# cure-lab/PnPInversion

Measured on AMD Instinct MI355X. Metric: edited images/sec @ 512x512, 50 DDIM-inv + 50 denoise steps, higher is better.
Workload: dtype f16 (fp32 accumulate; latents / scheduler math fp32); 1 GPU; single 512x512 image per rank, SD-1.x (seeded synthetic weights), directinversion+p2p, faithful schedule: 650 UNet sample-forwards + 1 VAE encode + 5 VAE decodes per image, Refine+Reweight+LocalBlend controller; text K/V projected once per loop (not per forward); ddim_steps=50, schedule=lockstep

## Files before the change

pnpinversion_amd/csrc/api.hip:

```cpp
#include <math.h>
#include <stdio.h>
#include <stdlib.h>
#include <string.h>

#include <algorithm>
#include <functional>
#include <memory>
#include <string>

#include "model.h"

static int g_text_kv = 1;
static int g_temb_cache = 1;

static int fail(pnpi_ctx* c, int status, const char* what) {
  c->err = what;
  return status;
}
static int fail_launch(pnpi_ctx* c, int code, const char* what) {
  char buf[640];
  if (code > 0) {
    snprintf(buf, sizeof(buf), "HIP error %d (%s) in %s", code, hipGetErrorString((hipError_t)code), what);
    c->err = buf;
    return PNPI_EHIP;
// ... 587 lines not shown
    half_t* f = talloc(c, (size_t)M * t.I);
    CK(op_gemm(c, h2, H, M, H, L.fc1.w, H, t.I, L.fc1.b, nullptr, 0, f, t.I));
    if (!c->dry) CK(launch_quick_gelu(f, (size_t)M * t.I, c->st));
    CK(op_gemm(c, f, t.I, M, t.I, L.fc2.w, t.I, H, L.fc2.b, x1, H, x, H));
    c->temp.release(mk);
  }
  half_t* y = palloc(c, (size_t)M * H);
  if (!c->dry) {
    PROF(PNPI_KC_LAYERNORM, 0.0, 2.0 * M * (double)H * 2.0, launch_layernorm(x, M, H, 1e-5f, t.final_ln.g, t.final_ln.b, y, c->st));
    CK(launch_f16_to_f32(y, (size_t)M * H, out, c->st));
  }
  return 0;
}

int pnpi_text_encode(pnpi_ctx* c, const int32_t* input_ids, int n, float* hidden_out) {
  if (!c || !input_ids || !hidden_out || n <= 0) return PNPI_EINVAL;
  CKP(check_clip_ready(c));
  if (n > c->rows_ident_n) return fail(c, PNPI_EINVAL, "more prompts than max(max_unet_rows, 8)");
  return clip_fwd(c, (const int*)input_ids, n, hidden_out);
}

static int conv_hook(pnpi_ctx* c, const void* x1, const void* x2, int C1, int C2, int B, int H, int W, int ksize, int stride, int pad, int ups,
                     int Ho, int Wo, const void* w, const float* bias, const void* res, int N, void* out, int force_cfg, int force_split,
                     float* stats_out, int* tile_rows_out) {
  GemmP p; gemm_defaults(p);
  p.x1 = (const half_t*)x1; p.x2 = (const half_t*)x2; p.C1 = C1; p.C2 = C2; p.ldx1 = C1; p.ldx2 = C2;
  p.B = B; p.H = H; p.W = W; p.Ho = Ho; p.Wo = Wo; p.ksize = ksize; p.stride = stride; p.pad = pad; p.ups = ups;
  p.K = ksize * ksize * (C1 + C2); p.w = (const half_t*)w; p.ldw = p.K; p.M = B * Ho * Wo; p.N = N;
  p.bias = bias; p.res = (const half_t*)res; p.ldres = N; p.out = (half_t*)out; p.ldo = N; p.stats = stats_out;
  CK(launch_igemm(p, c->splitk_ws, c->splitk_bytes, c->st, force_cfg, force_split, nullptr, tile_rows_out));
  return 0;
}
int pnpi_op_conv(pnpi_ctx* c, const void* x1, const void* x2, int C1, int C2, int B, int H, int W, int ksize, int stride, int pad,
                 int ups, int Ho, int Wo, const void* w, const float* bias, const void* res, int N, void* out, int force_cfg,
                 int force_split) {
  return conv_hook(c, x1, x2, C1, C2, B, H, W, ksize, stride, pad, ups, Ho, Wo, w, bias, res, N, out, force_cfg, force_split, nullptr, nullptr);
}
int pnpi_op_conv_stats(pnpi_ctx* c, const void* x1, const void* x2, int C1, int C2, int B, int H, int W, int ksize, int stride, int pad,
                       int ups, int Ho, int Wo, const void* w, const float* bias, const void* res, int N, void* out, int force_cfg,
                       int force_split, float* stats_out, int* tile_rows_out) {
  if (!c || !stats_out || !tile_rows_out) return PNPI_EINVAL;
  return conv_hook(c, x1, x2, C1, C2, B, H, W, ksize, stride, pad, ups, Ho, Wo, w, bias, res, N, out, force_cfg, force_split, stats_out, tile_rows_out);
}
int pnpi_tile_table_lookup(int M, int N, int K, int ksize, int* cfg, int* split, int* entry_m) {
  return igemm_table_lookup(M, N, K, ksize, cfg, split, entry_m);
}
int pnpi_set_tuning(const char* key, int value) {
  if (!key) return PNPI_EINVAL;
  if (!strcmp(key, "text_kv")) { g_text_kv = value; return 0; }
  if (!strcmp(key, "temb_cache")) { g_temb_cache = value; return 0; }
  if (!strcmp(key, "gn_inline_rows")) { norm_set_tuning_gn_inline_rows(value); return 0; }
  if (!strcmp(key, "attn_vt_perm")) { g_vt_perm = value; return 0; }
  if (!strcmp(key, "attn_aug")) { g_attn_aug = value; return 0; }
  if (!strcmp(key, "attn_pipe")) return attn_set_tuning_pipe(value) == 0 ? 0 : PNPI_EINVAL;
  if (!strcmp(key, "gn_slab")) { g_gn_slab = value; return 0; }
  if (!strcmp(key, "op_attention_aug")) { g_op_attention_aug = value; return 0; }
  if (!strcmp(key, "op_attention_vt_perm")) { g_op_attention_vt_perm = value; return 0; }
  if (!strcmp(key, "attn_bwd_flash")) { g_attn_bwd_flash = value; return 0; }
  return igemm_set_tuning(key, value) == 0 ? 0 : PNPI_EINVAL;
}
int pnpi_op_gemm(pnpi_ctx* c, const void* a, int lda, const void* w, int ldw, int M, int N, int K, float alpha, const float* bias,
                 const void* res, void* out, int ldo, int vt_col0, void* outT, int vt_ld, int vt_f32, int rpb, int force_cfg,
                 int force_split) {
  GemmP p; gemm_defaults(p);
  p.x1 = (const half_t*)a; p.C1 = K; p.ldx1 = lda; p.B = 1; p.H = 1; p.W = M; p.Ho = 1; p.Wo = M; p.ksize = 1;
  p.w = (const half_t*)w; p.ldw = ldw; p.M = M; p.N = N; p.K = K; p.alpha = alpha; p.bias = bias; p.res = (const half_t*)res;
  p.ldres = N; p.out = (half_t*)out; p.ldo = ldo;
  if (outT) { p.outT = outT; p.vt_col0 = vt_col0; p.vt_ld = vt_ld; p.vt_f32 = vt_f32; p.rows_per_batch = rpb; }
  CK(launch_igemm(p, c->splitk_ws, c->splitk_bytes, c->st, force_cfg, force_split));
  return 0;
}
int pnpi_op_gemm_geglu(pnpi_ctx* c, const void* a, int lda, const void* w, int ldw, int M, int N, int K, const float* bias, void* out,
                       int ldo) {
  GemmP p; gemm_defaults(p);
  p.x1 = (const half_t*)a; p.C1 = K; p.ldx1 = lda; p.B = 1; p.H = 1; p.W = M; p.Ho = 1; p.Wo = M; p.ksize = 1;
  p.w = (const half_t*)w; p.ldw = ldw; p.M = M; p.N = N; p.K = K; p.bias = bias; p.out = (half_t*)out; p.ldo = ldo; p.geglu = 1;
  CK(launch_igemm(p, c->splitk_ws, c->splitk_bytes, c->st));
  return 0;
}
int pnpi_op_groupnorm(pnpi_ctx* c, const void* x1, const void* x2, int C1, int C2, int B, int HW, int G, float eps, const float* gamma,
                      const float* beta, int silu, void* out) {
  CK(launch_groupnorm((const half_t*)x1, (const half_t*)x2, C1, C2, B, HW, G, eps, gamma, beta, silu, (half_t*)out, c->gn_partial, c->st));
  return 0;
}
int pnpi_op_layernorm(pnpi_ctx* c, const void* x, int M, int C, float eps, const float* gamma, const float* beta, void* out) {
  CK(launch_layernorm((const half_t*)x, M, C, eps, gamma, beta, (half_t*)out, c->st));
  return 0;
}
int pnpi_op_geglu(pnpi_ctx* c, const void* x, int M, int inner, void* out) {
  CK(launch_geglu((const half_t*)x, M, inner, (half_t*)out, c->st));
  return 0;
}
int pnpi_op_softmax_rows(pnpi_ctx* c, void* x, int M, int N, int ld) {
  CK(launch_softmax_rows((half_t*)x, M, N, ld, c->st));
  return 0;
}
int pnpi_op_attention_bwd(pnpi_ctx* c, const void* q, int ldq, int q_off, const void* k, int ldk, int k_off, const void* v, int ldv, int v_off,
                          const void* d_o, int ldo, int heads, int Nq, int Nk, int Dp, int dh, float scale, int B, void* dq, void* dk, void* dv,
                          void* scratch, size_t scratch_bytes) {
  if (!c || !q || !k || !v || !d_o || !dq || !dk || !dv) return PNPI_EINVAL;
  CKP(attn_bwd(c, (const half_t*)q, ldq, q_off, (const half_t*)k, ldk, k_off, (const half_t*)v, ldv, v_off, (const half_t*)d_o, ldo,
               heads, Nq, Nk, Dp, dh, scale, B, (half_t*)dq, (half_t*)dk, (half_t*)dv, scratch, scratch_bytes));
  return 0;
}
size_t pnpi_op_attention_bwd_scratch_bytes(int Nq, int Nk, int dh) { return attn_bwd_scratch_bytes(Nq, Nk, dh); }
int pnpi_op_layernorm_bwd(pnpi_ctx* c, const void* x, const void* dy, int M, int C, float eps, const float* gamma, void* dx) {
// ... 1 lines not shown
  return 0;
}
int pnpi_op_groupnorm_bwd(pnpi_ctx* c, const void* x1, const void* x2, int C1, int C2, int B, int HW, int G, float eps, const float* gamma,
                          const float* beta, int silu, const void* dy, void* dx) {
  const int C = C1 + C2;
  if (!(C & 7) && !(C1 & 7) && G <= 64) {
    float* ws = nullptr;
    CKP(gn_bwd_workspace(c, B, HW, G, &ws));
    CK(launch_groupnorm_bwd2((const half_t*)x1, (const half_t*)x2, C1, C2, B, HW, G, eps, gamma, beta, silu, (const half_t*)dy,
                             GnbOut{(half_t*)dx, C, 0}, GnbOut{(half_t*)dx + C1, C, 0}, ws, c->st));
    return 0;
  }
  CK(launch_groupnorm_bwd((const half_t*)x1, (const half_t*)x2, C1, C2, B, HW, G, eps, gamma, beta, silu, (const half_t*)dy, (half_t*)dx, c->st));
  return 0;
}
int pnpi_op_geglu_bwd(pnpi_ctx* c, const void* h, const void* dy, int M, int inner, void* dh) {
  CK(launch_geglu_bwd((const half_t*)h, (const half_t*)dy, M, inner, (half_t*)dh, c->st));
  return 0;
}
int pnpi_op_softmax_bwd_rows(pnpi_ctx* c, const float* P, const float* dP, int R, int N, int ld, float scale, void* dS) {
  CK(launch_softmax_bwd_rows(P, dP, (size_t)R, N, ld, scale, (half_t*)dS, c->st));
  return 0;
}
int pnpi_op_accumulate(pnpi_ctx* c, void* dst, const void* src, size_t n) {
  CK(launch_accumulate_f16((half_t*)dst, (const half_t*)src, n, c->st));
  return 0;
}
int pnpi_op_sumpool2x2(pnpi_ctx* c, const void* dup, int B, int H, int W, int C, void* dx) {
  CK(launch_sumpool2x2((const half_t*)dup, B, H, W, C, (half_t*)dx, c->st));
  return 0;
}
int pnpi_op_zero_stuff2(pnpi_ctx* c, const void* dy, int B, int Ho, int Wo, int C, void* out) {
  CK(launch_zero_stuff2((const half_t*)dy, B, Ho, Wo, C, (half_t*)out, c->st));
  return 0;
}
int pnpi_op_repack_dgrad(pnpi_ctx* c, const void* w, int N, int taps, int Cin, void* wd) {
  CK(launch_repack_dgrad((const half_t*)w, N, N, taps, Cin, (half_t*)wd, c->st));
  return 0;
}
int pnpi_op_null_text_loss(pnpi_ctx* c, const float* eps_u, const float* eps_c, const float* x, const float* target, int n, float w, float c_x,
                           float c_e, float grad_scale, void* d_eps_u, float* loss) {
  CK(launch_null_text_loss(eps_u, eps_c, x, target, n, w, c_x, c_e, grad_scale, (float*)d_eps_u, loss, c->st));
  return 0;
}
int pnpi_op_adam_step(pnpi_ctx* c, float* p, float* m, float* v, const float* g, int n, int k, float lr, float inv_scale) {
  CK(launch_adam_step(p, m, v, g, n, k, lr, inv_scale, c->st));
  return 0;
}
int pnpi_op_attention(pnpi_ctx* c, const void* q, int ldq, int q_off, const void* k, int ldk, int k_off, const void* vt, int ldv,
                      void* o, int ldo, int heads, int Nq, int Nk, int Dp, int dh, float scale, const int* rows_dev, int nrows) {
  AttnP a; a.q = (const half_t*)q; a.ldq = ldq; a.q_off = q_off; a.k = (const half_t*)k; a.ldk = ldk; a.k_off = k_off;
  a.vt = (const half_t*)vt; a.ldv = ldv; a.o = (half_t*)o; a.ldo = ldo; a.heads = heads; a.Nq = Nq; a.Nk = Nk; a.Dp = Dp; a.dh = dh;
  a.scale = scale; a.rows = rows_dev; a.nrows = nrows;
  a.vt_perm = (g_op_attention_vt_perm && attn_flash_uses_dma64(Dp, Nk, 0)) ? 1 : 0;
  a.aug = g_op_attention_aug;
  CK(launch_attn_flash(a, c->st));
  return 0;
}
int pnpi_op_cross_edit(pnpi_ctx* c, const void* q, int ldq, int q_off, const void* k, int ldk, int k_off, const void* vt, int ldv,
                       void* o, int ldo, int heads, int Nq, int Nk, int Dp, int dh, float scale, const int* pairs_dev, int npairs,
                       const void* mmatT, const float* c1, const float* c2, const float* lb_alpha, float* lb_acc, int lb_slot0,
                       int lb_nslots) {
  CrossEditP e; e.q = (const half_t*)q; e.ldq = ldq; e.q_off = q_off; e.k = (const half_t*)k; e.ldk = ldk; e.k_off = k_off;
  e.vt = (const half_t*)vt; e.ldv = ldv; e.o = (half_t*)o; e.ldo = ldo; e.heads = heads; e.Nq = Nq; e.Nk = Nk; e.Dp = Dp; e.dh = dh;
  e.scale = scale; e.pairs = pairs_dev; e.npairs = npairs; e.mmatT = (const half_t*)mmatT; e.c1 = c1; e.c2 = c2;
  e.lb_alpha = lb_alpha; e.lb_acc = lb_acc; e.lb_slot0 = lb_slot0; e.lb_nslots = lb_nslots; e.write_src = 1;
  CK(launch_attn_cross_edit(e, c->st));
  return 0;
}
int pnpi_op_local_blend(pnpi_ctx* c, const float* lb_acc, int nslots, int map_hw, int lat_hw, int C, float th, float* latents, int nimg) {
  CK(launch_local_blend(lb_acc, nslots, map_hw, lat_hw, C, th, latents, nimg, c->st));
  return 0;
}
int pnpi_op_local_blend_sub(pnpi_ctx* c, const float* lb_acc, int nslots, int map_hw, int lat_hw, int C, float th, float th_sub,
                            float* latents, int nimg) {
  CK(launch_local_blend(lb_acc, nslots, map_hw, lat_hw, C, th, latents, nimg, c->st, 4, th_sub));
  return 0;
}

#include "api_loops.inc"

}
```

pnpinversion_amd/csrc/api_graph.inc:

```
static void prof_open(pnpi_ctx* c, ProfRec& r) {
  (void)hipEventCreate(&r.a); (void)hipEventCreate(&r.b);
  (void)hipEventRecord(r.a, c->st);
}
static void prof_close(pnpi_ctx* c, ProfRec& r, int cls, double flops, double bytes, int M = 0, int N = 0, int K = 0, int ks = 0) {
  (void)hipEventRecord(r.b, c->st);
  r.cls = cls; r.flops = flops; r.bytes = bytes; r.M = M; r.N = N; r.K = K; r.ksize = ks;
  c->prof.push_back(r);
}
static int g_gn_slab = 0;
static int flush_pending(pnpi_ctx* c) {
  if (!c->pend_on) return 0;
  c->pend_on = false;
  return launch_splitk_reduce(c->pend, c->st);
}
#define PROF(cls, flops, bytes, expr) PROFD(cls, flops, bytes, 0, 0, 0, expr)
#define PROFD(cls, flops, bytes, d0, d1, d2, expr)            \
  do {                                                        \
    if (c->pend_on) { int _f = flush_pending(c); if (_f) return fail_launch(c, _f, "deferred split-K combine"); } \
    if (c->prof_on && !c->dry) {                              \
      ProfRec _pr; prof_open(c, _pr);                         \
      int _r = (expr);                                        \
      prof_close(c, _pr, (cls), (flops), (bytes), (d0), (d1), (d2)); \
      if (_r) return fail_launch(c, _r, #expr);               \
    } else {                                                  \
// ... 173 lines not shown
  if (!keep_acts(c)) c->temp.release(mk);
  return 0;
}

static int attn_materialized(pnpi_ctx* c, const half_t* q, int ldq, int q_off, const half_t* k, int ldk, int k_off, const half_t* vt, int ldv,
                             half_t* o, int ldo, int heads, int Nq, int Nk, int Dp, int dh, float scale, int B, int is_cross, int place,
                             int layer) {
  const int ldp = round_up_i(Nk, 8);
  const size_t need = align_up((size_t)B * heads * Nq * Nk * sizeof(float), 256);
  if (!c->attn_buf || need + (size_t)Nq * ldp * sizeof(half_t) > c->attn_buf_bytes)
    return fail(c, PNPI_ENOMEM, "attention callback buffer too small for this site (rows*heads*Nq*Nk floats + Nq*Nk halfs)");
  half_t* p16 = reinterpret_cast<half_t*>(reinterpret_cast<char*>(c->attn_buf) + need);
  for (int b = 0; b < B; ++b)
    for (int h = 0; h < heads; ++h) {
      float* S = c->attn_buf + ((size_t)b * heads + h) * Nq * Nk;
      VtOut v; v.outT = S; v.col0 = 0; v.ld = Nk; v.f32 = 1; v.rpb = Nk;
      CK(op_gemm(c, k + (size_t)b * Nk * ldk + k_off + h * Dp, ldk, Nk, Dp, q + (size_t)b * Nq * ldq + q_off + h * Dp, ldq, Nq, nullptr,
                 nullptr, 0, nullptr, Nq, scale, &v));
    }
  CK(launch_softmax_rows_f32(c->attn_buf, (size_t)B * heads * Nq, Nk, c->st));
  CKH(hipStreamSynchronize(c->st));
  if (c->attn_cb(c->attn_cb_user, c->attn_buf, B, heads, Nq, Nk, is_cross, place, layer)) return fail(c, PNPI_ESTATE, "attention callback failed");
  for (int b = 0; b < B; ++b)
    for (int h = 0; h < heads; ++h) {
      const float* S = c->attn_buf + ((size_t)b * heads + h) * Nq * Nk;
      CK(launch_f32_rows_to_f16_padded(S, Nq, Nk, ldp, p16, c->st));
      CK(op_gemm(c, p16, ldp, Nq, ldp, vt + ((size_t)b * heads + h) * Dp * (size_t)ldv, ldv, dh, nullptr, nullptr, 0,
                 o + (size_t)b * Nq * ldo + h * dh, ldo));
    }
  return 0;
}

static int transformer_fwd(pnpi_ctx* c, const TransformerW& t, const half_t* x, int B, int H, int W, const half_t* ctx16,
                           bool use_ctrl, int cur_step, half_t* out, Stats sx = Stats(), Stats* so = nullptr) {
  const pnpi_model_config& g = c->cfg;
  const size_t mk = c->temp.mark();
  const int block_index = c->tf_index++;
  const int C = t.C, N = H * W, M = B * N, hd = t.heads * t.Dp, X = g.cross_dim, T = g.ctx_len;
  const float scale = 1.0f / sqrtf((float)t.dh);
  CtrlDev& cd = c->cd;
  const bool edit = use_ctrl && cd.any_edit;

  half_t* g0 = talloc(c, (size_t)M * C);
  CK(op_gn(c, x, nullptr, C, 0, B, N, t.gn, g.norm_groups, 1e-6f, 0, g0, sx));
  half_t* hs = talloc(c, (size_t)M * C);
  CK(op_conv(c, g0, C, nullptr, 0, B, H, W, t.proj_in, 1, 0, 0, t.proj_in.b, nullptr, hs, H, W));

  half_t* n1 = talloc(c, (size_t)M * C);
  if (!c->dry) PROF(PNPI_KC_LAYERNORM, 0.0, 2.0 * M * (double)C * 2.0, launch_layernorm(hs, M, C, 1e-5f, t.ln1.g, t.ln1.b, n1, c->st));
  half_t* qk = talloc(c, (size_t)M * 2 * hd);
  const int ldv = round_up_i(N, 8);
  half_t* vt = talloc(c, (size_t)B * hd * ldv);
  if (c->attn_cb && !c->dry && ldv != N) CKH(hipMemsetAsync(vt, 0, (size_t)B * hd * ldv * sizeof(half_t), c->st));
  const int vperm = (g_vt_perm && !c->attn_cb && N % 16 == 0 && attn_flash_uses_dma64(t.Dp, N, 0)) ? 1 : 0;
  {
    VtOut v; v.outT = vt; v.col0 = 2 * hd; v.ld = ldv; v.f32 = 0; v.rpb = N; v.perm16 = vperm;
    CK(op_gemm(c, n1, C, M, C, t.w_qkv, C, 3 * hd, t.b_qkv_aug, nullptr, 0, qk, 2 * hd, 1.f, &v, 2.0 * M * 3.0 * C * C));
  }
  half_t* ao = talloc(c, (size_t)M * C);
  {
    AttnP a; a.q = qk; a.ldq = 2 * hd; a.q_off = 0; a.k = qk; a.ldk = 2 * hd; a.k_off = hd; a.vt = vt; a.ldv = ldv; a.vt_perm = vperm;
    a.aug = (t.b_qkv_aug && g_attn_aug) ? 1 : 0;
    a.o = ao; a.ldo = C; a.heads = t.heads; a.Nq = N; a.Nk = N; a.Dp = t.Dp; a.dh = t.dh; a.scale = scale;
    const bool rep = edit && cur_step >= cd.self_lo && cur_step < cd.self_hi && N <= cd.self_max_tokens;
    const bool masa_step = cd.masa_step_list ? (cur_step >= 0 && cur_step < (int)cd.masa_step_on.size() && cd.masa_step_on[cur_step]) : cur_step >= cd.masa_start_step;
    const bool masa_layer = cd.masa_layer_mask ? ((cd.masa_layer_mask >> block_index) & 1u) != 0 && block_index < 31 : block_index >= cd.masa_start_layer;
    const bool masa = use_ctrl && cd.masa_any && masa_step && masa_layer;
    a.rows = rep ? cd.rows_rep : (masa ? cd.rows_masa : cd.rows_id); a.nrows = B;
    c->ctr.executed_attn_flops += 4.0 * B * t.heads * (double)N * N * t.Dp;
    if (c->attn_cb && !c->dry) {
      CKP(attn_materialized(c, qk, 2 * hd, 0, qk, 2 * hd, hd, vt, ldv, ao, C, t.heads, N, N, t.Dp, t.dh, scale, B, 0, t.place, 2 * block_index));
    } else if (!c->dry) PROFD(PNPI_KC_ATTN_FLASH, 4.0 * B * t.heads * (double)N * N * t.dh, 0.0, N, N, t.Dp, launch_attn_flash(a, c->st));
  }
  half_t* hs1 = talloc(c, (size_t)M * C);
  CK(op_gemm(c, ao, C, M, C, t.o1.w, C, C, t.o1.b, hs, C, hs1, C));

  half_t* n2 = talloc(c, (size_t)M * C);
  if (!c->dry) PROF(PNPI_KC_LAYERNORM, 0.0, 2.0 * M * (double)C * 2.0, launch_layernorm(hs1, M, C, 1e-5f, t.ln2.g, t.ln2.b, n2, c->st));
  half_t* q2 = talloc(c, (size_t)M * hd);
  CK(op_gemm(c, n2, C, M, C, t.w_q2, C, hd, nullptr, nullptr, 0, q2, hd, 1.f, nullptr, 2.0 * M * (double)C * C));
  const int ldv2 = round_up_i(T, 8);
  half_t *k2, *vt2;
  if (c->tkv.use) {
    k2 = c->tkv.k[block_index]; vt2 = c->tkv.vt[block_index];
  } else {
    k2 = talloc(c, (size_t)B * T * hd);
    vt2 = talloc(c, (size_t)B * hd * ldv2);
    if (c->attn_cb && !c->dry && ldv2 != T) CKH(hipMemsetAsync(vt2, 0, (size_t)B * hd * ldv2 * sizeof(half_t), c->st));
    VtOut v; v.outT = vt2; v.col0 = hd; v.ld = ldv2; v.f32 = 0; v.rpb = T;
    CK(op_gemm(c, ctx16, X, B * T, X, t.w_kv2, X, 2 * hd, nullptr, nullptr, 0, k2, hd, 1.f, &v, 2.0 * B * T * 2.0 * C * X));
  }
  half_t* ao2 = talloc(c, (size_t)M * C);
  {
    AttnP a; a.q = q2; a.ldq = hd; a.q_off = 0; a.k = k2; a.ldk = hd; a.k_off = 0; a.vt = vt2; a.ldv = ldv2;
    a.o = ao2; a.ldo = C; a.heads = t.heads; a.Nq = N; a.Nk = T; a.Dp = t.Dp; a.dh = t.dh; a.scale = scale;
    a.rows = edit ? cd.rows_plain : cd.rows_id; a.nrows = edit ? cd.n_plain : B;
    c->ctr.executed_attn_flops += 4.0 * B * t.heads * (double)N * 96 * t.Dp;
    if (c->attn_cb && !c->dry) {
      CKP(attn_materialized(c, q2, hd, 0, k2, hd, 0, vt2, ldv2, ao2, C, t.heads, N, T, t.Dp, t.dh, scale, B, 1, t.place, 2 * block_index + 1));
    } else if (!c->dry) PROFD(PNPI_KC_ATTN_FLASH, 4.0 * a.nrows * t.heads * (double)N * T * t.dh, 0.0, N, T, t.Dp, launch_attn_flash(a, c->st));
    if (edit && !c->dry && !c->attn_cb) {
      CrossEditP e; e.q = q2; e.ldq = hd; e.q_off = 0; e.k = k2; e.ldk = hd; e.k_off = 0; e.vt = vt2; e.ldv = ldv2;
      e.o = ao2; e.ldo = C; e.heads = t.heads; e.Nq = N; e.Nk = T; e.Dp = t.Dp; e.dh = t.dh; e.scale = scale;
      e.pairs = cd.pairs; e.npairs = cd.npairs; e.mmatT = cd.mmatT;
      int srow = cur_step < cd.n_alpha_rows ? cur_step : cd.n_alpha_rows - 1;
      e.c1 = cd.coef + ((size_t)srow * 2 + 0) * cd.npairs * 96;
      e.c2 = cd.coef + ((size_t)srow * 2 + 1) * cd.npairs * 96;
// ... 379 lines not shown
```

pnpinversion_amd/csrc/attn.hip:

```cpp
#include <stdlib.h>

#include "ops.h"

static constexpr int KV_TILE = 64;
static constexpr int SV_LD = KV_TILE + 4;

template <int DP, bool PF>
__global__ void __launch_bounds__(256) attn_flash_kernel(AttnP p) {
  constexpr int KS = DP / 16;
  constexpr int OT = DP / 32;
  constexpr int SK_LD = DP + 8;
  __shared__ __attribute__((aligned(16))) half_t sK[KV_TILE * SK_LD];
  __shared__ __attribute__((aligned(16))) half_t sV[DP * SV_LD];

  const int tid = threadIdx.x, lane = tid & 63, wave = tid >> 6;
  const int h = lane >> 5, ql = lane & 31;
  const int nqt = (p.Nq + 127) >> 7, T = nqt * p.heads * p.nrows, per = (T + 7) >> 3;
  const int tix = (int)(blockIdx.x & 7) * per + (int)(blockIdx.x >> 3);
  if (tix >= T) return;
  const int qt = tix % nqt, head = (tix / nqt) % p.heads;
  const int* rw = p.rows + (tix / (nqt * p.heads)) * 4;
  const int orow = rw[0], qrow = rw[1], krow = rw[2], vrow = rw[3];
  const int qtok = qt * 128 + wave * 32 + ql;
  const bool qok = qtok < p.Nq;
// ... 104 lines not shown
    }
    const float mc = mrun * c;
    float psum = 0.f;
    half8 pf[2][2];
#pragma unroll
    for (int st = 0; st < 2; ++st)
#pragma unroll
      for (int r = 0; r < 16; ++r) {
        float pv = __builtin_amdgcn_exp2f(__builtin_fmaf(s[st][r], c, -mc));
        psum += pv;
        pf[st][r >> 3][r & 7] = (half_t)pv;
      }
    lrun += psum;
#pragma unroll
    for (int ot = 0; ot < OT; ++ot) {
#pragma unroll
      for (int st = 0; st < 2; ++st)
#pragma unroll
        for (int t = 0; t < 2; ++t) {
          const half_t* vb = sV + (ot * 32 + ql) * SV_LD + st * 32 + t * 16 + 4 * h;
          half4 lo = *reinterpret_cast<const half4*>(vb);
          half4 hi = *reinterpret_cast<const half4*>(vb + 8);
          half8 vf = {lo[0], lo[1], lo[2], lo[3], hi[0], hi[1], hi[2], hi[3]};
          O[ot] = mfma32(vf, pf[st][t], O[ot]);
        }
    }
  }
  const float ltot = lrun + __shfl_xor(lrun, 32, 64);
  const float inv = 1.f / ltot;
  if (p.lse && qok && h == 0) p.lse[((size_t)orow * p.heads + head) * p.Nq + qtok] = mrun * c + __log2f(ltot);
  if (qok) {
    half_t* op = p.o + ((size_t)orow * p.Nq + qtok) * p.ldo + head * p.dh;
#pragma unroll
    for (int ot = 0; ot < OT; ++ot)
#pragma unroll
      for (int g = 0; g < 4; ++g) {
        int d = ot * 32 + 8 * g + 4 * h;
        if (d + 3 < p.dh) {
          half4 o4 = {(half_t)(O[ot][4 * g] * inv), (half_t)(O[ot][4 * g + 1] * inv), (half_t)(O[ot][4 * g + 2] * inv),
                      (half_t)(O[ot][4 * g + 3] * inv)};
          *reinterpret_cast<half4*>(op + d) = o4;
        } else {
#pragma unroll
          for (int j = 0; j < 4; ++j)
            if (d + j < p.dh) op[d + j] = (half_t)(O[ot][4 * g + j] * inv);
        }
      }
  }
}

typedef __attribute__((address_space(3))) void* lds_ptr_t;
typedef const __attribute__((address_space(1))) void* gbl_ptr_t;

template <bool VPERM, int KSQ = 4, bool AUG = false>
__global__ void __launch_bounds__(256) attn_flash_dma64_kernel(AttnP p) {
  constexpr int DP = 64, KS = 4, OT = 2;
  constexpr int STAGE = 2 * 64 * 128;
  __shared__ __attribute__((aligned(1024))) char smem[2 * STAGE];

  const int tid = threadIdx.x, lane = tid & 63;
  const int wave = __builtin_amdgcn_readfirstlane(tid >> 6);
  const int h = lane >> 5, ql = lane & 31;
  const int nqt = (p.Nq + 127) >> 7, T = nqt * p.heads * p.nrows, per = (T + 7) >> 3;
  const int tix = (int)(blockIdx.x & 7) * per + (int)(blockIdx.x >> 3);
  if (tix >= T) return;
  const int qt = tix % nqt, head = (tix / nqt) % p.heads;
  const int* rw = p.rows + (tix / (nqt * p.heads)) * 4;
  const int orow = rw[0], qrow = rw[1], krow = rw[2], vrow = rw[3];
  const int qtok = qt * 128 + wave * 32 + ql;
  const bool qok = qtok < p.Nq;

  half8 qf[KSQ];
  {
    const half_t* qp = p.q + ((size_t)qrow * p.Nq + (qok ? qtok : 0)) * p.ldq + p.q_off + head * DP + h * 8;
#pragma unroll
    for (int ks = 0; ks < KSQ; ++ks) qf[ks] = qok ? ldg_half8(qp + ks * 16) : zero_half8();
  }
  const float c = p.scale * 1.44269504088896340736f;
  if (AUG) {
#pragma unroll
    for (int ks = 0; ks < KSQ; ++ks)
#pragma unroll
      for (int j = 0; j < 8; ++j) qf[ks][j] = (half_t)((float)qf[ks][j] * c);
  }
  floatx16 O[OT];
#pragma unroll
  for (int ot = 0; ot < OT; ++ot)
#pragma unroll
    for (int r = 0; r < 16; ++r) O[ot][r] = 0.f;
  float mrun = AUG ? 0.f : -INFINITY, lrun = 0.f;

  const half_t* kptr[2];
  const half_t* vptr[2];
#pragma unroll
  for (int i = 0; i < 2; ++i) {
    const int j = wave * 2 + i;
    const int line = 4 * (j & 1) + (lane >> 4);
    const int R = (j >> 1) * 16 + ((lane >> 3) & 1) * 8 + line;
    const int ch = (lane & 7) ^ line;
    kptr[i] = p.k + ((size_t)krow * p.Nk + R) * p.ldk + p.k_off + head * DP + ch * 8;
    vptr[i] = p.vt + (((size_t)vrow * p.heads + head) * DP + R) * (size_t)p.ldv + ch * 8;
  }
  auto issue = [&](int buf, int kv0) {
    char* sK = smem + buf * STAGE;
    char* sV = sK + 64 * 128;
#pragma unroll
    for (int i = 0; i < 2; ++i) {
      __builtin_amdgcn_global_load_lds((gbl_ptr_t)(kptr[i] + (size_t)kv0 * p.ldk), (lds_ptr_t)(sK + (wave * 2 + i) * 1024), 16, 0, 0);
      __builtin_amdgcn_global_load_lds((gbl_ptr_t)(vptr[i] + kv0), (lds_ptr_t)(sV + (wave * 2 + i) * 1024), 16, 0, 0);
    }
  };
  const int x7 = ql & 7;
  const int lane_row_off = (ql >> 4) * 2048 + (ql & 7) * 256 + ((ql >> 3) & 1) * 128;

  const int ntiles = p.Nk / 64;
  issue(0, 0);
  for (int it = 0; it < ntiles; ++it) {
    const int buf = it & 1;
    asm volatile("s_waitcnt vmcnt(0)" ::: "memory");
    __builtin_amdgcn_s_barrier();
    if (it + 1 < ntiles) issue(buf ^ 1, (it + 1) * 64);
    const char* sK = smem + buf * STAGE + lane_row_off;
    const char* sV = sK + 64 * 128;

    floatx16 s[2];
#pragma unroll
    for (int st = 0; st < 2; ++st) {
#pragma unroll
      for (int r = 0; r < 16; ++r) s[st][r] = 0.f;
#pragma unroll
      for (int ks = 0; ks < KSQ; ++ks) {
        half8 kf = *reinterpret_cast<const half8*>(sK + st * 4096 + (((ks * 2 + h) ^ x7) * 16));
        s[st] = mfma32(kf, qf[ks], s[st]);
      }
    }
    float mloc = s[0][0];
#pragma unroll
    for (int st = 0; st < 2; ++st)
#pragma unroll
      for (int r = 0; r < 16; ++r) mloc = fmaxf(mloc, s[st][r]);
    mloc = fmaxf(mloc, __shfl_xor(mloc, 32, 64));
    half8 pf[2][2];
    float psum = 0.f;
    if (AUG) {
      const bool grow = it == 0 || mloc > 8.0f;
      float delta = 0.f;
      if (__any(grow)) {
        const float target = mrun + ((it == 0 || mloc > 0.f) ? mloc : 0.f);
        const half_t mh = (half_t)target;
        const float mnew = (float)mh;
        delta = mnew - mrun;
        const float alpha = __builtin_amdgcn_exp2f(-delta);
#pragma unroll
        for (int ot = 0; ot < OT; ++ot)
#pragma unroll
          for (int r = 0; r < 16; ++r) O[ot][r] *= alpha;
        mrun = mnew;
        if (h == 1) qf[2][0] = (half_t)(-mnew);
#pragma unroll
        for (int st = 0; st < 2; ++st)
#pragma unroll
          for (int r = 0; r < 16; ++r) s[st][r] -= delta;
      }
#pragma unroll
      for (int st = 0; st < 2; ++st)
#pragma unroll
        for (int r = 0; r < 16; ++r) pf[st][r >> 3][r & 7] = (half_t)__builtin_amdgcn_exp2f(s[st][r]);
    } else {
    const bool grow = (mloc - mrun) * c > 8.0f;
    if (__any(grow)) {
      const float mnew = fmaxf(mrun, mloc);
      const float alpha = __builtin_amdgcn_exp2f((mrun - mnew) * c);
      lrun *= alpha;
#pragma unroll
      for (int ot = 0; ot < OT; ++ot)
#pragma unroll
        for (int r = 0; r < 16; ++r) O[ot][r] *= alpha;
      mrun = mnew;
    }
    const float mc = mrun * c;
#pragma unroll
    for (int st = 0; st < 2; ++st)
#pragma unroll
      for (int r = 0; r < 16; ++r) {
        float pv = __builtin_amdgcn_exp2f(__builtin_fmaf(s[st][r], c, -mc));
        psum += pv;
        pf[st][r >> 3][r & 7] = (half_t)pv;
      }
    }
    lrun += psum;
#pragma unroll
    for (int ot = 0; ot < OT; ++ot) {
#pragma unroll
      for (int st = 0; st < 2; ++st)
#pragma unroll
        for (int t = 0; t < 2; ++t) {
          const int c0 = st * 4 + t * 2;
          half8 vf;
          if (VPERM) {
            vf = *reinterpret_cast<const half8*>(sV + ot * 4096 + (((c0 + h) ^ x7) * 16));
          } else {
            half4 lo = *reinterpret_cast<const half4*>(sV + ot * 4096 + ((c0 ^ x7) * 16) + 8 * h);
            half4 hi = *reinterpret_cast<const half4*>(sV + ot * 4096 + (((c0 + 1) ^ x7) * 16) + 8 * h);
            vf = half8{lo[0], lo[1], lo[2], lo[3], hi[0], hi[1], hi[2], hi[3]};
          }
          O[ot] = mfma32(vf, pf[st][t], O[ot]);
        }
    }
  }
  float ltot;
  if (AUG) {
    const float lrow = O[1][4], lother = __shfl_xor(lrow, 32, 64);
    ltot = h == 0 ? lrow : lother;
  } else {
    ltot = lrun + __shfl_xor(lrun, 32, 64);
  }
  const float inv = 1.f / ltot;
  if (p.lse && qok && h == 0) p.lse[((size_t)orow * p.heads + head) * p.Nq + qtok] = (AUG ? mrun : mrun * c) + __log2f(ltot);
  if (qok) {
    half_t* op = p.o + ((size_t)orow * p.Nq + qtok) * p.ldo + head * p.dh;
#pragma unroll
    for (int ot = 0; ot < OT; ++ot)
#pragma unroll
      for (int g = 0; g < 4; ++g) {
        int d = ot * 32 + 8 * g + 4 * h;
        if (d + 3 < p.dh) {
          half4 o4 = {(half_t)(O[ot][4 * g] * inv), (half_t)(O[ot][4 * g + 1] * inv), (half_t)(O[ot][4 * g + 2] * inv),
                      (half_t)(O[ot][4 * g + 3] * inv)};
          *reinterpret_cast<half4*>(op + d) = o4;
        } else {
#pragma unroll
          for (int j = 0; j < 4; ++j)
            if (d + j < p.dh) op[d + j] = (half_t)(O[ot][4 * g + j] * inv);
        }
      }
  }
}

#ifdef PNPI_ABLATIONS
#define SGB(mask, n) __builtin_amdgcn_sched_group_barrier(mask, n, 0)
#define PIPE_SCHED()                                                     \
  do {                                                                   \
    SGB(0x100, 3);                                                       \
    SGB(0x008, 1); SGB(0x002, 4);                                        \
    SGB(0x008, 1); SGB(0x002, 4);                                        \
    SGB(0x008, 1); SGB(0x100, 2); SGB(0x002, 6);                         \
    SGB(0x008, 1); SGB(0x100, 2); SGB(0x002, 5);                         \
    SGB(0x008, 1); SGB(0x002, 5);                                        \
    SGB(0x008, 1); SGB(0x002, 5);                                        \
    SGB(0x008, 1); SGB(0x002, 8);                                        \
  } while (0)
template <int PLACE>
__global__ void __launch_bounds__(256) attn_flash_pipe64_kernel(AttnP p) {
  constexpr int DP = 64;
  constexpr int KT = 64 * 128;
  __shared__ __attribute__((aligned(1024))) char smem[4 * KT];
  const int tid = threadIdx.x, lane = tid & 63;
  const int wave = __builtin_amdgcn_readfirstlane(tid >> 6);
  const int h = lane >> 5, ql = lane & 31;
  const int nqt = (p.Nq + 127) >> 7, T = nqt * p.heads * p.nrows, per = (T + 7) >> 3;
  const int tix = (int)(blockIdx.x & 7) * per + (int)(blockIdx.x >> 3);
  if (tix >= T) return;
  const int qt = tix % nqt, head = (tix / nqt) % p.heads;
  const int* rw = p.rows + (tix / (nqt * p.heads)) * 4;
  const int orow = rw[0], qrow = rw[1], krow = rw[2], vrow = rw[3];
// ... 92 lines not shown
  else asm volatile("s_waitcnt vmcnt(2)" ::: "memory");
  __builtin_amdgcn_s_barrier();
  floatx16 sa = scores(0, 0), sb;
  float mloc = rowmax(sa);
  for (int it = 0; it < nt; ++it) {
    const int slot = it & 1;
    const bool more = it + 1 < nt;
    if (more) asm volatile("s_waitcnt vmcnt(2)" ::: "memory"); else asm volatile("s_waitcnt vmcnt(0)" ::: "memory");
    __builtin_amdgcn_s_barrier();
    if (more) issue_v(slot ^ 1, (it + 1) * 64);
    move_reference(sa, mloc, it == 0);
    sb = scores(slot, 1);
    exp_pv(sa, slot, 0);
    mloc = rowmax(sb);
    if (PLACE == 1) PIPE_SCHED();
    if (more) asm volatile("s_waitcnt vmcnt(2)" ::: "memory"); else asm volatile("s_waitcnt vmcnt(0)" ::: "memory");
    __builtin_amdgcn_s_barrier();
    if (it + 2 < nt) issue_k(slot, (it + 2) * 64);
    move_reference(sb, mloc, false);
    if (more) sa = scores(slot ^ 1, 0);
    exp_pv(sb, slot, 1);
    if (more) mloc = rowmax(sa);
    if (PLACE == 1) PIPE_SCHED();
  }
  const float lrow = O[1][4], lother = __shfl_xor(lrow, 32, 64);
  const float ltot = h == 0 ? lrow : lother;
  const float inv = 1.f / ltot;
  if (p.lse && qok && h == 0) p.lse[((size_t)orow * p.heads + head) * p.Nq + qtok] = mrun + __log2f(ltot);
  if (qok) {
    half_t* op = p.o + ((size_t)orow * p.Nq + qtok) * p.ldo + head * p.dh;
#pragma unroll
    for (int ot = 0; ot < 2; ++ot)
#pragma unroll
      for (int g = 0; g < 4; ++g) {
        const int d = ot * 32 + 8 * g + 4 * h;
        if (d + 3 < p.dh) {
          half4 o4 = {(half_t)(O[ot][4 * g] * inv), (half_t)(O[ot][4 * g + 1] * inv), (half_t)(O[ot][4 * g + 2] * inv), (half_t)(O[ot][4 * g + 3] * inv)};
          *reinterpret_cast<half4*>(op + d) = o4;
        } else {
#pragma unroll
          for (int j = 0; j < 4; ++j)
            if (d + j < p.dh) op[d + j] = (half_t)(O[ot][4 * g + j] * inv);
        }
      }
  }
}
static int g_attn_pipe = 0;
int attn_set_tuning_pipe(int v) { g_attn_pipe = v; return 0; }
#else
static const int g_attn_pipe = 0;
int attn_set_tuning_pipe(int v) { return v == 0 ? 0 : -2; }
#endif

bool attn_flash_uses_dma64(int Dp, int Nk, int causal) {
  static const bool no_dma = getenv("PNPI_ATTN_NODMA") != nullptr;
  return Dp == 64 && Nk % 64 == 0 && Nk >= 128 && !no_dma && !causal;
}

int launch_attn_flash(const AttnP& p, hipStream_t st) {
  if (p.nrows <= 0) return 0;
  if ((p.ldq & 7) || (p.ldk & 7) || (p.ldv & 7) || (p.q_off & 7) || (p.k_off & 7) || (p.dh & 3) || (p.ldo & 3)) return -3;
  const int total = ((p.Nq + 127) / 128) * p.heads * p.nrows;
  dim3 grid((unsigned)(((total + 7) / 8) * 8), 1, 1);
  static const bool no_dma = getenv("PNPI_ATTN_NODMA") != nullptr;
  if (p.Dp == 64 && p.Nk % 64 == 0 && p.Nk >= 128 && !no_dma && !p.causal) {
    static const bool ksq3 = !(getenv("PNPI_ATTN_KSQ4") != nullptr);
    static const bool no_aug = getenv("PNPI_ATTN_NOAUG") != nullptr;
    if (p.aug && p.dh == 40 && ksq3 && !no_aug) {
#ifdef PNPI_ABLATIONS
      if (p.vt_perm && g_attn_pipe == 1) attn_flash_pipe64_kernel<0><<<grid, 256, 0, st>>>(p);
      else if (p.vt_perm && g_attn_pipe == 2) attn_flash_pipe64_kernel<1><<<grid, 256, 0, st>>>(p);
      else
#endif
      if (p.vt_perm) attn_flash_dma64_kernel<true, 3, true><<<grid, 256, 0, st>>>(p);
      else attn_flash_dma64_kernel<false, 3, true><<<grid, 256, 0, st>>>(p);
    } else if (p.dh <= 48 && ksq3) {
      if (p.vt_perm) attn_flash_dma64_kernel<true, 3><<<grid, 256, 0, st>>>(p);
      else attn_flash_dma64_kernel<false, 3><<<grid, 256, 0, st>>>(p);
    } else {
      if (p.vt_perm) attn_flash_dma64_kernel<true><<<grid, 256, 0, st>>>(p);
      else attn_flash_dma64_kernel<false><<<grid, 256, 0, st>>>(p);
    }
    return (int)hipGetLastError();
  }
  if (p.vt_perm) return -6;
  const bool pf = p.Nk > 2 * KV_TILE;
#define LAUNCH_FLASH(D) (pf ? attn_flash_kernel<D, true><<<grid, 256, 0, st>>>(p) : attn_flash_kernel<D, false><<<grid, 256, 0, st>>>(p))
  switch (p.Dp) {
    case 32: LAUNCH_FLASH(32); break;
    case 64: LAUNCH_FLASH(64); break;
    case 96: LAUNCH_FLASH(96); break;
    case 128: LAUNCH_FLASH(128); break;
    case 160: LAUNCH_FLASH(160); break;
    default: return -5;
  }
#undef LAUNCH_FLASH
  return (int)hipGetLastError();
}

static constexpr int CE_KEYS = 96;
static constexpr int CE_LD = CE_KEYS + 4;

template <int DP>
__global__ void __launch_bounds__(256) attn_cross_edit_kernel(CrossEditP p) {
  constexpr int KS = DP / 16, OT = DP / 32, SK_LD = DP + 8;
  extern __shared__ __attribute__((aligned(16))) char smem_raw[];
  half_t* sK = reinterpret_cast<half_t*>(smem_raw);
  half_t* sV = sK + 2 * CE_KEYS * SK_LD;
  half_t* sM = sV + 2 * DP * CE_LD;
  float* sC = reinterpret_cast<float*>(sM + CE_KEYS * CE_LD);

  const int tid = threadIdx.x, lane = tid & 63, wave = tid >> 6;
  const int h = lane >> 5, ql = lane & 31;
  const int head = blockIdx.y, pair = blockIdx.z;
  const int rows2[2] = {p.pairs[pair * 2 + 0], p.pairs[pair * 2 + 1]};
  const int qtok = blockIdx.x * 128 + wave * 32 + ql;
  const bool qok = qtok < p.Nq;

  half8 qf2[2][KS];
#pragma unroll
  for (int which = 0; which < 2; ++which) {
// ... 508 lines not shown
```

pnpinversion_amd/csrc/ops.h:

```cpp
#pragma once
#include "common.h"

struct GemmP {
  const half_t* x1; const half_t* x2;
  int C1, C2, ldx1, ldx2;
  int B, H, W, Ho, Wo;
  int ksize, stride, pad, ups;
  const half_t* w; int ldw;
  int M, N, K;
  const float* bias;
  const half_t* res; int ldres;
  float alpha;
  half_t* out; int ldo;
  void* outT; int vt_col0, vt_ld, vt_f32, rows_per_batch;
  int vt_perm16;
  float* slab; int splitk, kchunks_per_split;
  float* stats;
  int geglu;
  int epi_lds;
  int bias_init;
  int res_late;
  int k_order;
  int gx, gy, gz, tile_order;
  int nbatch;
// ... 9 lines not shown
int igemm_set_tuning(const char* key, int value);
void igemm_set_dma(int on);

int launch_groupnorm(const half_t* x1, const half_t* x2, int C1, int C2, int B, int HW, int G, float eps,
                     const float* gamma, const float* beta, int silu, half_t* out, float* partial, hipStream_t st);
int launch_groupnorm_fused(const half_t* x1, const half_t* x2, int C1, int C2, int B, int HW, int G, float eps,
                           const float* gamma, const float* beta, int silu, half_t* out, const float* st1, int tpb1,
                           const float* st2, int tpb2, float* scratch, hipStream_t st);
void norm_set_tuning_gn_inline_rows(int v);
struct GnSlab { const float* slab; int splitk; size_t stride; const float* bias; const half_t* res; int ldres; half_t* sum_out; };
bool groupnorm_slab_ok(int C1, int C2, int HW, int G);
int launch_groupnorm_slab(const GnSlab& sl, const half_t* x2, int C1, int C2, int B, int HW, int G, float eps, const float* gamma,
                          const float* beta, int silu, half_t* out, hipStream_t st);
int launch_layernorm(const half_t* x, int M, int C, float eps, const float* gamma, const float* beta, half_t* out,
                     hipStream_t st);
int launch_geglu(const half_t* x, int M, int I, half_t* out, hipStream_t st);
int launch_softmax_rows(half_t* x, int M, int N, int ld, hipStream_t st);
int launch_softmax_rows_f32(float* x, size_t M, int N, hipStream_t st);
int launch_f32_rows_to_f16_padded(const float* in, size_t M, int N, int ld, half_t* out, hipStream_t st);
int launch_gemv(const float* x, int K, const half_t* W, int N, const float* bias, const float* bias2, int silu_in,
                float* out, hipStream_t st);
int launch_repack_matrix(const void* src, int src_f16, int rows, int cols, int taps, half_t* dst, int dst_ld, int cin_pad,
                         int row0, int dh, int Dp, hipStream_t st, int ilv_half = 0);
int launch_repack_vec(const void* src, int src_f16, int n, float* dst, hipStream_t st, int ilv_half = 0);
int launch_nchw_f32_to_nhwc_f16(const float* in, int B, int C, int HW, int Cp, half_t* out, hipStream_t st);
int launch_f32_to_f16(const float* in, size_t n, half_t* out, hipStream_t st);
int launch_img_u8_to_nhwc(const uint8_t* img, int n, int HW, int Cp, half_t* out, hipStream_t st);
int launch_dec_to_u8(const float* nchw, int n, int HW, uint8_t* out_hwc, hipStream_t st);
int launch_scale_f32(const float* in, size_t n, float s, float* out, hipStream_t st);
int launch_gather_rows_f32(const float* in, const int* rows, int nrows, size_t row_elems, float* out, hipStream_t st);
int launch_embed_tokens(const int* ids, int M, int T, int H, int vocab, const half_t* tok_emb, const half_t* pos_emb, half_t* out,
                        hipStream_t st);
int launch_quick_gelu(half_t* x, size_t n, hipStream_t st);
int launch_f16_to_f32(const half_t* in, size_t n, float* out, hipStream_t st);

__host__ __device__ inline int vt_perm16_pos(int tok) { return tok ^ ((((tok >> 2) ^ (tok >> 3)) & 1) ? 12 : 0); }

struct AttnP {
  const half_t* q; int ldq, q_off;
  const half_t* k; int ldk, k_off;
  const half_t* vt; int ldv;
  half_t* o; int ldo;
  int heads, Nq, Nk, Dp, dh;
  float scale;
  const int* rows;
  int nrows;
  int causal = 0;
  int vt_perm = 0;
  int aug = 0;
  float* lse = nullptr;
};
int launch_attn_flash(const AttnP& p, hipStream_t st);
int attn_set_tuning_pipe(int v);
bool attn_flash_uses_dma64(int Dp, int Nk, int causal);

struct BwdMat { const half_t* p; long hs; int ld; int w; };
struct AttnBwdP {
  BwdMat b1, b2;
  BwdMat l1, l2;
  int nb, nl, heads;
  float scale;
  float* lse;
  float* dsum;
  half_t* out; long out_hs; int out_ld, out_w;
  const half_t* o = nullptr; long o_hs = 0; int o_ld = 0;
  int nsplit = 1;
  float* part = nullptr;
};
int launch_attn_bwd_reduce(const AttnBwdP& p, hipStream_t st);
int launch_attn_bwd_flash(const AttnBwdP& p, int mode , int Dp, hipStream_t st);

struct CrossEditP {
  const half_t* q; int ldq, q_off;
  const half_t* k; int ldk, k_off;
  const half_t* vt; int ldv;
  half_t* o; int ldo;
  int heads, Nq, Nk, Dp, dh;
  float scale;
  const int* pairs;
  int npairs;
  const half_t* mmatT;
  const float* c1; const float* c2;
  const float* lb_alpha;
  float* lb_acc;
  int lb_planes = 2;
  int lb_slot0, lb_nslots;
  int write_src;
};
int launch_attn_cross_edit(const CrossEditP& p, hipStream_t st);

int launch_ddim_move(const float* x, const float* eps, float a_from, float a_to, size_t n, float* out, hipStream_t st);
int launch_ddim_prev_recon(const float* x, const float* eps, float a_from, float a_to, const float* ref, float lr, const float* mask, size_t n,
                           float* out, float* x0_out, hipStream_t st);
struct CfgStepP {
  const float* eps = nullptr;
  const float* x = nullptr; float* x_out = nullptr;
  int nimg = 0, rows_per_img = 1; size_t row_elems = 0;
  float gscale = 1.f, a_t = 1.f, a_prev = 1.f;
  const float* noise_loss = nullptr; int offset_rows = 0;
  const float* target = nullptr; float offset_scale = 1.f; float* offset_out = nullptr;
  const float* prox_thr = nullptr; int prox_mode = 0;
  const float *recon_ref = nullptr, *inv_ref = nullptr;
  float recon_lr = 0.f; int dilate = 0, lat_h = 0, lat_w = 0;
};
int launch_cfg_ddim_prev(const CfgStepP& p, hipStream_t st);
int launch_quantile_abs_diff(const float* eps, int nimg, int rows_per_img, size_t row_elems, float q, float* thr_out, hipStream_t st);
int launch_fill_f32(float* p, int n, float v, hipStream_t st);
// ... 34 lines not shown
```

Baseline: 1.025 images/s.

## Extend DMA flash-attention kernel to padded head widths 96 and 160

Generalizes the global-to-LDS DMA flash attention kernel over the padded head width, adding 96- and 160-column variants (with the augmented-softmax trick for dh=80) and a dynamic-LDS launch for 160. Attention layers with larger heads previously fell back to the slower non-DMA path. These layers can now use asynchronous direct loads and double buffering, and V-transpose permutation is allowed for them too. The wider tiles raise LDS use per block, which can reduce occupancy, and the new address swizzles for the extra 32-column slab add complexity.

```diff
diff --git a/pnpinversion_amd/csrc/api.hip b/pnpinversion_amd/csrc/api.hip
--- a/pnpinversion_amd/csrc/api.hip
+++ b/pnpinversion_amd/csrc/api.hip
@@ -663,6 +663,7 @@
   if (!strcmp(key, "gn_inline_rows")) { norm_set_tuning_gn_inline_rows(value); return 0; }
   if (!strcmp(key, "attn_vt_perm")) { g_vt_perm = value; return 0; }
   if (!strcmp(key, "attn_aug")) { g_attn_aug = value; return 0; }
+  if (!strcmp(key, "attn_wide_dma")) { attn_set_tuning_wide_dma(value); return 0; }
   if (!strcmp(key, "attn_pipe")) return attn_set_tuning_pipe(value) == 0 ? 0 : PNPI_EINVAL;
   if (!strcmp(key, "gn_slab")) { g_gn_slab = value; return 0; }
   if (!strcmp(key, "op_attention_aug")) { g_op_attention_aug = value; return 0; }
@@ -770,7 +771,7 @@
   AttnP a; a.q = (const half_t*)q; a.ldq = ldq; a.q_off = q_off; a.k = (const half_t*)k; a.ldk = ldk; a.k_off = k_off;
   a.vt = (const half_t*)vt; a.ldv = ldv; a.o = (half_t*)o; a.ldo = ldo; a.heads = heads; a.Nq = Nq; a.Nk = Nk; a.Dp = Dp; a.dh = dh;
   a.scale = scale; a.rows = rows_dev; a.nrows = nrows;
-  a.vt_perm = (g_op_attention_vt_perm && attn_flash_uses_dma64(Dp, Nk, 0)) ? 1 : 0;
+  a.vt_perm = (g_op_attention_vt_perm && attn_flash_uses_dma(Dp, Nk, 0)) ? 1 : 0;
   a.aug = g_op_attention_aug;
   CK(launch_attn_flash(a, c->st));
   return 0;
diff --git a/pnpinversion_amd/csrc/api_graph.inc b/pnpinversion_amd/csrc/api_graph.inc
--- a/pnpinversion_amd/csrc/api_graph.inc
+++ b/pnpinversion_amd/csrc/api_graph.inc
@@ -249,7 +249,7 @@
   const int ldv = round_up_i(N, 8);
   half_t* vt = talloc(c, (size_t)B * hd * ldv);
   if (c->attn_cb && !c->dry && ldv != N) CKH(hipMemsetAsync(vt, 0, (size_t)B * hd * ldv * sizeof(half_t), c->st));
-  const int vperm = (g_vt_perm && !c->attn_cb && N % 16 == 0 && attn_flash_uses_dma64(t.Dp, N, 0)) ? 1 : 0;
+  const int vperm = (g_vt_perm && !c->attn_cb && N % 16 == 0 && attn_flash_uses_dma(t.Dp, N, 0)) ? 1 : 0;
   {
     VtOut v; v.outT = vt; v.col0 = 2 * hd; v.ld = ldv; v.f32 = 0; v.rpb = N; v.perm16 = vperm;
     CK(op_gemm(c, n1, C, M, C, t.w_qkv, C, 3 * hd, t.b_qkv_aug, nullptr, 0, qk, 2 * hd, 1.f, &v, 2.0 * M * 3.0 * C * C));
diff --git a/pnpinversion_amd/csrc/attn.hip b/pnpinversion_amd/csrc/attn.hip
--- a/pnpinversion_amd/csrc/attn.hip
+++ b/pnpinversion_amd/csrc/attn.hip
@@ -180,11 +180,24 @@
 typedef __attribute__((address_space(3))) void* lds_ptr_t;
 typedef const __attribute__((address_space(1))) void* gbl_ptr_t;
 
-template <bool VPERM, int KSQ = 4, bool AUG = false>
+template <bool VPERM, int KSQ = 4, bool AUG = false, int DP = 64>
 __global__ void __launch_bounds__(256) attn_flash_dma64_kernel(AttnP p) {
-  constexpr int DP = 64, KS = 4, OT = 2;
-  constexpr int STAGE = 2 * 64 * 128;
-  __shared__ __attribute__((aligned(1024))) char smem[2 * STAGE];
+  static_assert(DP % 32 == 0 && KSQ * 16 <= DP, "head widths are whole 32-column output tiles");
+  constexpr int OT = DP / 32;
+  constexpr int NP64 = DP / 64;
+  constexpr int KTILE = 64 * DP * 2;
+  constexpr int STAGE = 2 * KTILE;
+  constexpr int NPW = DP / 32;
+  constexpr int AUGD = DP == 64 ? 40 : 80;
+  static_assert(!AUG || (DP == 64 && KSQ == 3) || (DP == 96 && KSQ == 6), "AUG needs a padding column inside the k-steps that run");
+  char* smem;
+  if constexpr (2 * STAGE <= 64 * 1024) {
+    __shared__ __attribute__((aligned(1024))) char smem_static[2 * STAGE];
+    smem = smem_static;
+  } else {
+    extern __shared__ __attribute__((aligned(1024))) char smem_dynamic[];
+    smem = smem_dynamic;
+  }
 
   const int tid = threadIdx.x, lane = tid & 63;
   const int wave = __builtin_amdgcn_readfirstlane(tid >> 6);
@@ -218,28 +231,36 @@
     for (int r = 0; r < 16; ++r) O[ot][r] = 0.f;
   float mrun = AUG ? 0.f : -INFINITY, lrun = 0.f;
 
-  const half_t* kptr[2];
-  const half_t* vptr[2];
-#pragma unroll
-  for (int i = 0; i < 2; ++i) {
-    const int j = wave * 2 + i;
+  const half_t* kptr[NPW];
+  const half_t* vptr[NPW];
+#pragma unroll
+  for (int i = 0; i < NPW; ++i) {
+    const int j = wave * NPW + i;
     const int line = 4 * (j & 1) + (lane >> 4);
     const int R = (j >> 1) * 16 + ((lane >> 3) & 1) * 8 + line;
     const int ch = (lane & 7) ^ line;
-    kptr[i] = p.k + ((size_t)krow * p.Nk + R) * p.ldk + p.k_off + head * DP + ch * 8;
+    if constexpr (DP == 64) {
+      kptr[i] = p.k + ((size_t)krow * p.Nk + R) * p.ldk + p.k_off + head * DP + ch * 8;
+    } else {
+      const int Rk = j < 8 * NP64 ? ((j & 7) >> 1) * 16 + ((lane >> 3) & 1) * 8 + line : (j - 8 * NP64) * 16 + (lane >> 2);
+      const int ck = j < 8 * NP64 ? (j >> 3) * 64 + ch * 8 : NP64 * 64 + (((lane & 3) ^ ((Rk >> 2) & 3)) * 8);
+      kptr[i] = p.k + ((size_t)krow * p.Nk + Rk) * p.ldk + p.k_off + head * DP + ck;
+    }
     vptr[i] = p.vt + (((size_t)vrow * p.heads + head) * DP + R) * (size_t)p.ldv + ch * 8;
   }
   auto issue = [&](int buf, int kv0) {
     char* sK = smem + buf * STAGE;
-    char* sV = sK + 64 * 128;
-#pragma unroll
-    for (int i = 0; i < 2; ++i) {
-      __builtin_amdgcn_global_load_lds((gbl_ptr_t)(kptr[i] + (size_t)kv0 * p.ldk), (lds_ptr_t)(sK + (wave * 2 + i) * 1024), 16, 0, 0);
-      __builtin_amdgcn_global_load_lds((gbl_ptr_t)(vptr[i] + kv0), (lds_ptr_t)(sV + (wave * 2 + i) * 1024), 16, 0, 0);
+    char* sV = sK + KTILE;
+#pragma unroll
+    for (int i = 0; i < NPW; ++i) {
+      __builtin_amdgcn_global_load_lds((gbl_ptr_t)(kptr[i] + (size_t)kv0 * p.ldk), (lds_ptr_t)(sK + (wave * NPW + i) * 1024), 16, 0, 0);
+      __builtin_amdgcn_global_load_lds((gbl_ptr_t)(vptr[i] + kv0), (lds_ptr_t)(sV + (wave * NPW + i) * 1024), 16, 0, 0);
     }
   };
   const int x7 = ql & 7;
   const int lane_row_off = (ql >> 4) * 2048 + (ql & 7) * 256 + ((ql >> 3) & 1) * 128;
+  const int lane_row32_off = ql * 64 - lane_row_off;
+  const int x3 = (ql >> 2) & 3;
 
   const int ntiles = p.Nk / 64;
   issue(0, 0);
@@ -249,7 +270,7 @@
     __builtin_amdgcn_s_barrier();
     if (it + 1 < ntiles) issue(buf ^ 1, (it + 1) * 64);
     const char* sK = smem + buf * STAGE + lane_row_off;
-    const char* sV = sK + 64 * 128;
+    const char* sV = sK + KTILE;
 
     floatx16 s[2];
 #pragma unroll
@@ -258,7 +279,10 @@
       for (int r = 0; r < 16; ++r) s[st][r] = 0.f;
 #pragma unroll
       for (int ks = 0; ks < KSQ; ++ks) {
-        half8 kf = *reinterpret_cast<const half8*>(sK + st * 4096 + (((ks * 2 + h) ^ x7) * 16));
+        half8 kf;
+        if constexpr (DP == 64) kf = *reinterpret_cast<const half8*>(sK + st * 4096 + (((ks * 2 + h) ^ x7) * 16));
+        else if ((ks >> 2) < NP64) kf = *reinterpret_cast<const half8*>(sK + (ks >> 2) * 8192 + st * 4096 + ((((ks & 3) * 2 + h) ^ x7) * 16));
+        else kf = *reinterpret_cast<const half8*>(sK + NP64 * 8192 + lane_row32_off + st * 2048 + ((((ks & 3) * 2 + h) ^ x3) * 16));
         s[st] = mfma32(kf, qf[ks], s[st]);
       }
     }
@@ -284,7 +308,7 @@
 #pragma unroll
           for (int r = 0; r < 16; ++r) O[ot][r] *= alpha;
         mrun = mnew;
-        if (h == 1) qf[2][0] = (half_t)(-mnew);
+        if (h == (AUGD % 16) / 8) qf[AUGD / 16][0] = (half_t)(-mnew);
 #pragma unroll
         for (int st = 0; st < 2; ++st)
 #pragma unroll
@@ -338,7 +362,8 @@
   }
   float ltot;
   if (AUG) {
-    const float lrow = O[1][4], lother = __shfl_xor(lrow, 32, 64);
+    static_assert(AUGD % 8 == 0, "the row is the lower half-wave's first accumulator of a group of four");
+    const float lrow = O[AUGD / 32][(AUGD % 32) / 2], lother = __shfl_xor(lrow, 32, 64);
     ltot = h == 0 ? lrow : lother;
   } else {
     ltot = lrun + __shfl_xor(lrun, 32, 64);
@@ -537,9 +562,22 @@
 int attn_set_tuning_pipe(int v) { return v == 0 ? 0 : -2; }
 #endif
 
-bool attn_flash_uses_dma64(int Dp, int Nk, int causal) {
+static int g_attn_wide_dma = 1;
+void attn_set_tuning_wide_dma(int v) { g_attn_wide_dma = v; }
+bool attn_flash_uses_dma(int Dp, int Nk, int causal) {
   static const bool no_dma = getenv("PNPI_ATTN_NODMA") != nullptr;
-  return Dp == 64 && Nk % 64 == 0 && Nk >= 128 && !no_dma && !causal;
+  if (Nk % 64 != 0 || no_dma || causal) return false;
+  return Dp == 64 ? Nk >= 128 : ((Dp == 96 || Dp == 160) && g_attn_wide_dma);
+}
+
+template <bool VPERM, int KSQ, bool AUG>
+static int launch_dma160(const AttnP& p, dim3 grid, hipStream_t st) {
+  auto kern = attn_flash_dma64_kernel<VPERM, KSQ, AUG, 160>;
+  constexpr int LDS = 2 * 2 * 64 * 160 * 2;
+  static const hipError_t attr = hipFuncSetAttribute((const void*)kern, hipFuncAttributeMaxDynamicSharedMemorySize, LDS);
+  if (attr != hipSuccess) return (int)attr;
+  kern<<<grid, 256, LDS, st>>>(p);
+  return 0;
 }
 
 int launch_attn_flash(const AttnP& p, hipStream_t st) {
@@ -547,11 +585,24 @@
   if ((p.ldq & 7) || (p.ldk & 7) || (p.ldv & 7) || (p.q_off & 7) || (p.k_off & 7) || (p.dh & 3) || (p.ldo & 3)) return -3;
   const int total = ((p.Nq + 127) / 128) * p.heads * p.nrows;
   dim3 grid((unsigned)(((total + 7) / 8) * 8), 1, 1);
-  static const bool no_dma = getenv("PNPI_ATTN_NODMA") != nullptr;
-  if (p.Dp == 64 && p.Nk % 64 == 0 && p.Nk >= 128 && !no_dma && !p.causal) {
-    static const bool ksq3 = !(getenv("PNPI_ATTN_KSQ4") != nullptr);
-    static const bool no_aug = getenv("PNPI_ATTN_NOAUG") != nullptr;
-    if (p.aug && p.dh == 40 && ksq3 && !no_aug) {
+  static const bool ksq3 = !(getenv("PNPI_ATTN_KSQ4") != nullptr);
+  static const bool no_aug = getenv("PNPI_ATTN_NOAUG") != nullptr;
+  if (attn_flash_uses_dma(p.Dp, p.Nk, p.causal) && (p.Dp == 64 || !p.lse)) {
+    if (p.Dp == 96) {
+      if (p.aug && p.dh == 80 && ksq3 && !no_aug) {
+        if (p.vt_perm) attn_flash_dma64_kernel<true, 6, true, 96><<<grid, 256, 0, st>>>(p);
+        else attn_flash_dma64_kernel<false, 6, true, 96><<<grid, 256, 0, st>>>(p);
+      } else if (p.dh <= 80 && ksq3) {
+        if (p.vt_perm) attn_flash_dma64_kernel<true, 5, false, 96><<<grid, 256, 0, st>>>(p);
+        else attn_flash_dma64_kernel<false, 5, false, 96><<<grid, 256, 0, st>>>(p);
+      } else {
+        if (p.vt_perm) attn_flash_dma64_kernel<true, 6, false, 96><<<grid, 256, 0, st>>>(p);
+        else attn_flash_dma64_kernel<false, 6, false, 96><<<grid, 256, 0, st>>>(p);
+      }
+    } else if (p.Dp == 160) {
+      const int r = p.vt_perm ? launch_dma160<true, 10, false>(p, grid, st) : launch_dma160<false, 10, false>(p, grid, st);
+      if (r) return r;
+    } else if (p.aug && p.dh == 40 && ksq3 && !no_aug) {
 #ifdef PNPI_ABLATIONS
       if (p.vt_perm && g_attn_pipe == 1) attn_flash_pipe64_kernel<0><<<grid, 256, 0, st>>>(p);
       else if (p.vt_perm && g_attn_pipe == 2) attn_flash_pipe64_kernel<1><<<grid, 256, 0, st>>>(p);
diff --git a/pnpinversion_amd/csrc/ops.h b/pnpinversion_amd/csrc/ops.h
--- a/pnpinversion_amd/csrc/ops.h
+++ b/pnpinversion_amd/csrc/ops.h
@@ -85,7 +85,8 @@
 };
 int launch_attn_flash(const AttnP& p, hipStream_t st);
 int attn_set_tuning_pipe(int v);
-bool attn_flash_uses_dma64(int Dp, int Nk, int causal);
+void attn_set_tuning_wide_dma(int v);
+bool attn_flash_uses_dma(int Dp, int Nk, int causal);
 
 struct BwdMat { const half_t* p; long hs; int ld; int w; };
 struct AttnBwdP {
```

Result: no change. 1.033 images/s (median of 6 runs) (+0.8%).
